# openfheorg/openfhe-boolean-circuit-evaluator

Measured on NVIDIA B200. Metric: bootstrapped gates/sec (STD128_OPT GINX), higher is better.
Workload: dtype u32

## Files before the change

### openfhe-boolean-circuit-evaluator_b200/csrc/common.hpp

```cpp
#pragma once
#include <cstddef>
#include <cstdint>

namespace bfhe {

using u8 = uint8_t;
using u16 = uint16_t;
using u32 = uint32_t;
using u64 = uint64_t;
using i32 = int32_t;
using i64 = int64_t;

struct DevConst {
  u32 Q, Q2;
  u32 qinv_neg;
  u32 unused_mu;
  u32 oneM;
  u32 Q8;
  u32 n, N, q, factor;
  u32 qKS, baseKS, dKS;
  u32 baseR, dR, dG, logBG;
  u32 ct_stride;
  u32 ninv, ninvs;
  u32 nM, nMs;
  u32 gate_const[9];
  u32 reserved_[3];
  u32 tw[32], tws[32], itw[32], itws[32];
};

struct DevGate {
  const u32 *in0;
  const u32 *in1;
  u32 *out;
  u32 op;
  u32 pad;
};

enum : u32 { OP_OR = 0, OP_AND = 1, OP_NOR = 2, OP_NAND = 3, OP_XOR_FAST = 4, OP_XNOR_FAST = 5, OP_XOR = 6, OP_XNOR = 7,
             OP_BOOTSTRAP = 8, OP_NEG0 = 0x100, OP_NEG1 = 0x200 };

struct LaunchInfo {
  int gates_per_cta;
  int ctas;
  size_t smem_bytes;
};

struct V2Bufs {
  const u32 *d_bk4 = nullptr;
  const u32 *d_tw2 = nullptr;
  const u32 *d_F = nullptr;
  const u32 *d_bkx = nullptr;
  const u32 *d_twx = nullptr;
};

int launch_blind_rotate(const DevConst &P, int method_ap, const DevGate *d_gates, int count, const u32 *d_bk,
                        const u32 *d_twl , const u32 *d_psiM,
                        u32 *d_ext , u32 *d_acc_dbg , int force_gates_per_cta,
                        void *stream, LaunchInfo *info, const V2Bufs *v2 = nullptr);
bool v2_supported(const DevConst &P, int method_ap);
int v2_set_attrs();
int launch_bk_permute_v2(const u32 *d_src, u32 *d_dst, size_t npoly, void *stream);
int cl2_max_gates();
int launch_bk_split_cl4(const u32 *d_src, u32 *d_dst, size_t npoly, void *stream);
int launch_blind_rotate_cl2(const DevConst &P, const DevGate *d_gates, int count, const V2Bufs &vb, u32 *d_ext, u32 *d_acc_dbg,
                            void *stream, LaunchInfo *info);
bool clx_supported(const DevConst &P, int method_ap);
size_t clx_tw_words();
int clx_set_attrs();
int clx_max_gates();
int clx_fast_gates();
int launch_bk_slice_clx(const u32 *d_src, u32 *d_dst, size_t npoly, int method_ap, void *stream);
int launch_blind_rotate_clx(const DevConst &P, int method_ap, const DevGate *d_gates, int count, const V2Bufs &vb, u32 *d_ext,
                            u32 *d_acc_dbg, void *stream, LaunchInfo *info);
struct PeerX {
  u32 *const *slabs = nullptr;
  const u32 *local_base = nullptr;
  u32 *const *flags = nullptr;
  u32 *counter = nullptr;
  const u32 *epoch = nullptr;
  u32 world = 1, rank = 0, index = 0, per_epoch = 1;
};
int launch_keyswitch(const DevConst &P, const u32 *d_ext, const DevGate *d_gates, int count, const void *d_ksk,
                     int ksk_elem_bytes, void *stream, const PeerX *px = nullptr);
int launch_peer_epoch_bump(u32 *epoch, void *stream);
int launch_peer_wait(const u32 *local_flags, const u32 *epoch, u32 world, u32 rank, int index, u32 per_epoch, u32 *err, void *stream);
int launch_peer_signal(const PeerX &px, void *stream);
int launch_eval_not(const DevConst &P, const u32 *const *d_in, u32 *const *d_out, int count, void *stream);
int launch_bk_convert(const DevConst &P, const u32 *d_coef, u32 *d_dev, size_t npoly, const u32 *d_twl, void *stream);
int launch_dbg_ntt(const DevConst &P, const u32 *d_a, const u32 *d_b, u32 *d_rt, u32 *d_prod, int npoly, const u32 *d_twl,
                   void *stream);
int launch_microbench(int which, u32 *d_sink, int iters, int *threads_total, int *ops_per_thread_iter, void *stream);
int blind_rotate_set_attrs();

}
```

### openfhe-boolean-circuit-evaluator_b200/csrc/engine.cu

```cuda
#include "engine.hpp"
#include "device.cuh"
#include <algorithm>
#include <cstdio>
#include <cstring>
#include <omp.h>

using namespace bfhe;

namespace bfhe {
static thread_local std::string g_err;
void set_error(const std::string &msg) { g_err = msg; }
int cuda_fail(cudaError_t e, const char *what) {
  set_error(std::string("CUDA error: ") + cudaGetErrorString(e) + " in " + what);
  return BFHE_ERR_CUDA;
}
}

extern "C" const char *bfhe_last_error(void) { return g_err.c_str(); }

static constexpr double SIGMA = 3.19;
static const GaussTable &gauss_table() {
  static const GaussTable t(SIGMA);
  return t;
}
// ... 159 lines not shown
          for (u32 g = 0; g < 2; g++) putf(at(1, 2 + g), 256 + 64 * k + 2 * lane + g);
          for (u32 g = 0; g < 4; g++) putf(at(1, 4 + g), 512 + 128 * k + 4 * lane + g);
        }
        for (u32 s5 = 0; s5 < 5; s5++)
          for (u32 t = 0; t < 256; t++) puti(8 + 256 * (size_t)s5 + t, (512u >> s5) + ((256 * k + t) >> (s5 + 1)));
      }
      ok = cudaMalloc(&c->d_twx, tx.size() * 4) == cudaSuccess && cudaMemcpy(c->d_twx, tx.data(), tx.size() * 4, cudaMemcpyHostToDevice) == cudaSuccess;
      c->v2.d_twx = c->d_twx;
    }
    int sms = 148;
    cudaDeviceGetAttribute(&sms, cudaDevAttrMultiProcessorCount, device);
    c->chunk = std::max<size_t>(1, bfhe_ctx::CHUNK / (4 * (size_t)sms)) * 4 * (size_t)sms;
    if (c->chunk > bfhe_ctx::CHUNK) c->chunk = bfhe_ctx::CHUNK;
    if (!ok) {
      cuda_fail(cudaGetLastError(), "bfhe_create: device allocation");
      bfhe_destroy(c);
      return nullptr;
    }
  }
  return c;
}

extern "C" void bfhe_destroy(bfhe_ctx *c) {
  if (!c) return;
  if (c->device >= 0) {
    cudaSetDevice(c->device);
    cudaDeviceSynchronize();
    for (auto &s : c->spans) { cudaEventDestroy(s.a); cudaEventDestroy(s.b); }
    cudaFree(c->d_bk); cudaFree(c->d_twl); cudaFree(c->d_psiM); cudaFree(c->d_ksk); cudaFree(c->d_gates); cudaFree(c->d_ext);
    cudaFree(c->d_tmp); cudaFree(c->d_ptr_in); cudaFree(c->d_ptr_out); cudaFree(c->e2e_slab);
    cudaFree(c->d_gates_b); cudaFree(c->d_ext_b);
    cudaFree(c->d_bk4); cudaFree(c->d_tw2); cudaFree(c->d_F);
    cudaFree(c->d_bkx); cudaFree(c->d_twx);
    for (int i = 0; i < 2; i++) {
      if (c->ev_br[i]) cudaEventDestroy(c->ev_br[i]);
      if (c->ev_ks[i]) cudaEventDestroy(c->ev_ks[i]);
    }
    if (c->ks_stream) cudaStreamDestroy(c->ks_stream);
    for (int i = 0; i < 2; i++) {
      if (c->h_gates[i]) cudaFreeHost(c->h_gates[i]);
      if (c->stage_ev[i]) cudaEventDestroy(c->stage_ev[i]);
    }
    if (c->own_stream) cudaStreamDestroy(c->own_stream);
  }
  delete c;
}

extern "C" int bfhe_get_params(const bfhe_ctx *c, bfhe_params *out) {
  if (!c || !out) return BFHE_ERR_ARG;
  *out = c->p;
  return BFHE_OK;
}
extern "C" int bfhe_set_stream(bfhe_ctx *c, void *s, int use_own) {
  if (!c || c->device < 0) return BFHE_ERR_STATE;
  c->stream = use_own ? c->own_stream : (cudaStream_t)s;
  return BFHE_OK;
}
extern "C" int bfhe_sync(bfhe_ctx *c) {
  if (!c || c->device < 0) { set_error("no device attached"); return BFHE_ERR_CUDA; }
  BFHE_CUDA(cudaStreamSynchronize(c->stream));
  return BFHE_OK;
}

extern "C" int bfhe_keygen(bfhe_ctx *c, uint64_t seed) {
  if (!c) return BFHE_ERR_ARG;
  SeedKey key;
// ... 117 lines not shown
    const size_t npoly = c->bk_words / N, slice = 1 << 15;
    u32 *d_coef = nullptr;
    BFHE_CUDA(cudaMalloc(&d_coef, std::min(npoly, slice) * N * 4));
    for (size_t p0 = 0; p0 < npoly; p0 += slice) {
      const size_t np = std::min(slice, npoly - p0);
      BFHE_CUDA(cudaMemcpyAsync(d_coef, c->bk_coef.data() + p0 * N, np * N * 4, cudaMemcpyHostToDevice, c->stream));
      int rc = launch_bk_convert(c->P, d_coef, c->d_bk + p0 * N, np, c->d_twl, c->stream);
      if (rc) return cuda_fail((cudaError_t)rc, "bk_convert");
      BFHE_CUDA(cudaStreamSynchronize(c->stream));
    }
    cudaFree(d_coef);
  }
  cudaFree(c->d_bk4); c->d_bk4 = nullptr; c->v2.d_bk4 = nullptr;
  if (c->d_tw2 && v2_supported(c->P, p.method == BFHE_AP)) {
    u32 *tmp = nullptr;
    BFHE_CUDA(cudaMalloc(&tmp, c->bk_words * 4));
    int rc = launch_bk_permute_v2(c->d_bk, tmp, c->bk_words / N, c->stream);
    if (rc) { cudaFree(tmp); return cuda_fail((cudaError_t)rc, "bk_permute_v2"); }
    if (cudaMalloc(&c->d_bk4, c->bk_words * 4) != cudaSuccess) { cudaFree(tmp); return cuda_fail(cudaGetLastError(), "cudaMalloc(d_bk4)"); }
    rc = launch_bk_split_cl4(tmp, c->d_bk4, c->bk_words / N, c->stream);
    if (rc) { cudaFree(tmp); return cuda_fail((cudaError_t)rc, "bk_split_cl4"); }
    cudaStreamSynchronize(c->stream);
    cudaFree(tmp);
    c->v2.d_bk4 = c->d_bk4;
  }
  cudaFree(c->d_bkx); c->d_bkx = nullptr; c->v2.d_bkx = nullptr;
  if (c->d_twx && clx_supported(c->P, p.method == BFHE_AP)) {
    BFHE_CUDA(cudaMalloc(&c->d_bkx, c->bk_words * 4));
    int rc = launch_bk_slice_clx(c->d_bk, c->d_bkx, c->bk_words / N, p.method == BFHE_AP, c->stream);
    if (rc) return cuda_fail((cudaError_t)rc, "bk_slice_clx");
    BFHE_CUDA(cudaStreamSynchronize(c->stream));
    c->v2.d_bkx = c->d_bkx;
  }
  {
    const u32 rowlen = c->ksk_elem_bytes == 2 ? 512 : p.ct_stride;
    if (c->ksk_elem_bytes == 2 && p.n + 1 > 512) { set_error("LWE dimension too large for the packed key-switch kernel"); return BFHE_ERR_ARG; }
    const size_t rows = (size_t)N * p.baseKS * p.dKS, bytes = rows * rowlen * c->ksk_elem_bytes;
    std::vector<u8> dev(bytes, 0);
    const size_t src_row = (size_t)(p.n + 1) * c->ksk_elem_bytes, dst_row = (size_t)rowlen * c->ksk_elem_bytes;
#pragma omp parallel for schedule(static)
    for (i64 i = 0; i < (i64)N; i++)
      for (u32 j = 0; j < p.baseKS; j++)
        for (u32 k = 0; k < p.dKS; k++) {
          const size_t s = (((size_t)i * p.baseKS + j) * p.dKS + k), d = (((size_t)i * p.dKS + k) * p.baseKS + j);
          std::memcpy(dev.data() + d * dst_row, c->ksk.data() + s * src_row, src_row);
        }
    BFHE_CUDA(cudaMalloc(&c->d_ksk, bytes));
    BFHE_CUDA(cudaMemcpy(c->d_ksk, dev.data(), bytes, cudaMemcpyHostToDevice));
  }
  c->dev_keys = true;
  return BFHE_OK;
}

extern "C" size_t bfhe_keyblob_size(const bfhe_ctx *c) {
  if (!c) return 0;
  return sizeof(KeyBlobHeader) + pad8((size_t)c->p.n * 4) + pad8(c->bk_words * 4) + pad8(c->ksk_elems * c->ksk_elem_bytes);
}
extern "C" int bfhe_export_keys(const bfhe_ctx *c, void *buf, size_t cap, int include_sk) {
  if (!c || !buf) return BFHE_ERR_ARG;
  if (!c->has_bt) { set_error("no keys to export"); return BFHE_ERR_STATE; }
  if (cap < bfhe_keyblob_size(c)) { set_error("export buffer too small"); return BFHE_ERR_ARG; }
  KeyBlobHeader h{};
  std::memcpy(h.magic, "BFHEKEY1", 8);
  const bfhe_params &p = c->p;
  h.version = 1; h.paramset = p.paramset; h.method = p.method; h.n = p.n; h.N = p.N; h.q = p.q;
  h.baseKS = p.baseKS; h.dKS = p.dKS; h.baseG = p.baseG; h.dG = p.dG; h.baseR = p.baseR; h.dR = p.dR;
// ... 435 lines not shown
```

### openfhe-boolean-circuit-evaluator_b200/csrc/engine.hpp

```cpp
#pragma once
#include "../../include/bfhe.h"
#include "common.hpp"
#include "hostmath.hpp"
#include <cuda_runtime.h>
#include <mutex>
#include <string>
#include <vector>

namespace bfhe {

void set_error(const std::string &msg);
int cuda_fail(cudaError_t e, const char *what);
#define BFHE_CUDA(call)                                                                                                \
  do {                                                                                                                 \
    cudaError_t _e = (call);                                                                                           \
    if (_e != cudaSuccess) return ::bfhe::cuda_fail(_e, #call);                                                        \
  } while (0)

struct ProfSpan {
  cudaEvent_t a, b;
  int kernel;
};

}

struct bfhe_ctx {
  bfhe_params p{};
  bfhe::DevConst P{};
  int device = -1;
  cudaStream_t own_stream = nullptr, stream = nullptr;
  bfhe::u64 psi = 0;
  bfhe::HostNtt hntt;

  std::vector<bfhe::i32> sk;
  std::vector<bfhe::i32> z;
  bool has_sk = false, has_bt = false;
  bool ofhe_have_bk = false, ofhe_have_ksk = false;
  std::vector<bfhe::u32> bk_coef;
  std::vector<bfhe::u8> ksk;
  bfhe::u32 ksk_elem_bytes = 4;
  bfhe::u64 bk_words = 0, ksk_elems = 0;

  bfhe::u32 *d_bk = nullptr, *d_twl = nullptr, *d_psiM = nullptr;
  void *d_ksk = nullptr;
  bfhe::u32 *d_bk4 = nullptr, *d_tw2 = nullptr, *d_F = nullptr;
  bfhe::u32 *d_bkx = nullptr, *d_twx = nullptr;
  bfhe::V2Bufs v2{};
  bool dev_keys = false;

  static constexpr size_t CHUNK = 32768;
  size_t chunk = CHUNK;
  bfhe::DevGate *d_gates = nullptr;
  bfhe::DevGate *d_gates_b = nullptr;
  bfhe::u32 *d_ext_b = nullptr;
  cudaStream_t ks_stream = nullptr;
  cudaEvent_t ev_br[2] = {nullptr, nullptr}, ev_ks[2] = {nullptr, nullptr};
  bfhe::DevGate *h_gates[2] = {nullptr, nullptr};
  cudaEvent_t stage_ev[2] = {nullptr, nullptr};
  int stage_next = 0;
  bfhe::u32 *d_ext = nullptr;
  bfhe::u32 *d_tmp = nullptr;
  size_t tmp_rows = 0;
  const bfhe::u32 **d_ptr_in = nullptr;
  bfhe::u32 **d_ptr_out = nullptr;
  size_t ptr_cap = 0;
  bfhe::u32 *e2e_slab = nullptr;
  size_t e2e_rows = 0;
  int force_g = 0;
  double form_cost_ms[4] = {0, 0, 0, 0};
  bool form_cost_measured = false;

  bool profiling = false;
  std::vector<bfhe::ProfSpan> spans;
  std::mutex mtx;
};

namespace bfhe {
int run_gate_list(bfhe_ctx *c, const DevGate *host_list, size_t count, u32 *acc_dbg_host);
int ensure_device_keys(bfhe_ctx *c);
// ... 2 lines not shown
```

### openfhe-boolean-circuit-evaluator_b200/csrc/kernels.cu

```cuda
#include "device.cuh"
#include <type_traits>
#include <cuda_runtime.h>
#include <cstdlib>

namespace bfhe {

constexpr int SOL_LAT_WIDE = 0x05, SOL_LAT_NARROW = 0x0a;

__device__ __forceinline__ u32 f_phys(u32 u) { return (u & ~31u) | ((u ^ (u >> 5)) & 31u); }
template <int E> struct Lay {
  static constexpr int C = E / 4;
  __device__ __forceinline__ static int swz(int tp) { return E == 32 ? (tp & 7) : ((tp >> 1) & 3); }
  __device__ __forceinline__ static int chunk_off(int tp, int c) { return E * tp + 4 * (c ^ swz(tp)); }
  __device__ __forceinline__ static int elem_off(int k, int lane) {
    if (E == 32) return 32 * k + 4 * ((lane >> 2) ^ (k & 7)) + (lane & 3);
    int j = lane & 15;
    return 16 * (2 * k + (lane >> 4)) + 4 * ((j >> 2) ^ (k & 3)) + (j & 3);
  }
};
template <int E> __device__ __forceinline__ void row_load(const u32 *buf, u32 (&x)[E], int lane) {
#pragma unroll
  for (int c = 0; c < E / 4; c++) {
    uint4 v = *reinterpret_cast<const uint4 *>(buf + Lay<E>::chunk_off(lane, c));
    x[4 * c] = v.x; x[4 * c + 1] = v.y; x[4 * c + 2] = v.z; x[4 * c + 3] = v.w;
// ... 85 lines not shown
  int B = B0;
  for (int T = 1; T < E; T *= 2) {
    const int NB = 2 * B;
    const bool last = 2 * T >= E;
    B = (last ? NB > MAXLAST : NB > 16) ? 2 : NB;
  }
  return B;
}

struct TwTabs {
  const u32 *fw, *fws, *iw, *iws;
};

template <int LOGN, bool PRE = false, int SOLW = 0, int SOLN = 0>
__device__ __forceinline__ void ntt_forward(u32 (&x)[(1 << LOGN) / 32], u32 *buf, const DevConst &P, const TwTabs &tt, int lane,
                                            const u32 *pre = nullptr) {
  constexpr int E = (1 << LOGN) / 32;
  const u32 Q = P.Q, Q2 = P.Q2;
  ct_pass<E, true, SOLW, PRE>(x, P.tw, P.tws, Q, Q2, nullptr, nullptr, 0, pre);
  if constexpr (LOGN & 1) {
    const bool up = lane & 16;
#pragma unroll
    for (int k = 0; k < E; k++) {
      u32 v = up ? mul_shoup(x[k], P.tw[16 + k], P.tws[16 + k], Q) : x[k];
      u32 o = __shfl_xor_sync(0xffffffffu, v, 16);
      x[k] = up ? (o - v + Q2) : (v + o);
    }
  }
  __syncwarp();
  col_store<E>(buf, x, lane);
  __syncwarp();
  row_load<E>(buf, x, lane);
  ct_pass<E, false, SOLN>(x, P.tw, P.tws, Q, Q2, tt.fw, tt.fws, lane);
}

template <int LOGN, bool PRE = false>
__device__ __forceinline__ void ntt_forward2(u32 (&xa)[(1 << LOGN) / 32], u32 (&xb)[(1 << LOGN) / 32], u32 *bufa, u32 *bufb, const DevConst &P,
                                             const TwTabs &tt, int lane, const u32 *prea = nullptr, const u32 *preb = nullptr) {
  constexpr int E = (1 << LOGN) / 32;
  static_assert((LOGN & 1) == 0, "even log2 N only");
  const u32 Q = P.Q, Q2 = P.Q2;
  ct_pass<E, true, 0, PRE>(xa, P.tw, P.tws, Q, Q2, nullptr, nullptr, 0, prea);
  ct_pass<E, true, 0, PRE>(xb, P.tw, P.tws, Q, Q2, nullptr, nullptr, 0, preb);
  __syncwarp();
  col_store<E>(bufa, xa, lane);
  col_store<E>(bufb, xb, lane);
  __syncwarp();
  row_load<E>(bufa, xa, lane);
  row_load<E>(bufb, xb, lane);
  ct_pass<E, false>(xa, P.tw, P.tws, Q, Q2, tt.fw, tt.fws, lane);
  ct_pass<E, false>(xb, P.tw, P.tws, Q, Q2, tt.fw, tt.fws, lane);
}

template <int LOGN, int B0>
__device__ __forceinline__ void ntt_inverse(u32 (&x)[(1 << LOGN) / 32], u32 *buf, const DevConst &P, const TwTabs &tt, int lane) {
  constexpr int E = (1 << LOGN) / 32;
  const u32 Q = P.Q;
  constexpr int ML = (LOGN & 1) ? 8 : 16;
  GsRun<E, 1, B0, false, ML>::run(x, P.itw, P.itws, Q, tt.iw, tt.iws, lane);
  constexpr int B1 = gs_out_bound(E, B0, ML);
  __syncwarp();
  row_store<E>(buf, x, lane);
  __syncwarp();
  col_load<E>(buf, x, lane);
  if constexpr (LOGN & 1) {
    static_assert(B1 <= 8, "bound");
    const bool up = lane & 16;
    const u32 off = B1 * Q;
#pragma unroll
    for (int k = 0; k < E; k++) {
      u32 o = __shfl_xor_sync(0xffffffffu, x[k], 16);
      u32 D = o - x[k] + off;
      x[k] = up ? mul_shoup(D, P.itw[16 + k], P.itws[16 + k], Q) : (x[k] + o);
    }
    constexpr int B2 = 2 * B1;
    GsRun<E, 1, B2, true, 32>::run(x, P.itw, P.itws, Q);
  } else {
    GsRun<E, 1, B1, true, 32>::run(x, P.itw, P.itws, Q);
  }
#pragma unroll
  for (int k = 0; k < E; k++) x[k] = csub(lazy_reduce(x[k], Q), Q);
}

__device__ __forceinline__ u32 brev(u32 x, int bits) { return __brev(x) >> (32 - bits); }
template <int DG, int LOGBG> constexpr u32 digit_offset() {
  u32 off = 0;
  for (int l = 0; l < DG; l++) off += (1u << (LOGBG - 1)) << (LOGBG * l);
  return off;
}

template <int LOGN, int DG, int LOGBG, int G, bool AP> struct BrCfg {
  static constexpr int N = 1 << LOGN, E = N / 32, C = E / 4, ROWS = 2 * DG;
  static constexpr int W = 2 * G, THREADS = 32 * W;
  static constexpr int NPAD = AP ? 1024 : 512;
  static constexpr size_t dct_words = (size_t)G * ROWS * N;
  static constexpr bool LUT = (LOGBG == 7 && LOGN == 10);
  static constexpr size_t lut_words = LUT ? (size_t)32 << LOGBG : 0;
  static constexpr size_t smem_bytes = (dct_words + 4 * N + (AP ? 0 : 2 * N) + lut_words) * 4 + (size_t)G * NPAD * 2;
};

template <int LOGN, int DG, int LOGBG, int G, bool AP>
__global__ void __launch_bounds__(64 * G, 1)
blind_rotate_kernel(const __grid_constant__ DevConst P, const DevGate *__restrict__ gates, int count,
                    const u32 *__restrict__ bk, const u32 *__restrict__ g_twl, const u32 *__restrict__ g_psiM,
                    u32 *__restrict__ ext, u32 *__restrict__ acc_dbg) {
  using Cfg = BrCfg<LOGN, DG, LOGBG, G, AP>;
  constexpr int N = Cfg::N, E = Cfg::E, C = Cfg::C, ROWS = Cfg::ROWS, W = Cfg::W, NPAD = Cfg::NPAD;
  constexpr u32 DIGIT_OFF = digit_offset<DG, LOGBG>();
  extern __shared__ __align__(128) unsigned char smem_raw[];
  u32 *dct = reinterpret_cast<u32 *>(smem_raw);
  u32 *s_tw = dct + Cfg::dct_words;
  u32 *s_psiM = s_tw + 4 * N;
  u32 *s_lut = s_psiM + (AP ? 0 : 2 * N);
  u16 *s_idx = reinterpret_cast<u16 *>(s_lut + Cfg::lut_words);

  const int tid = threadIdx.x, lane = tid & 31, warp = tid >> 5;
  const int g = warp >> 1, c = warp & 1;
  if constexpr (Cfg::LUT) {
    for (int i = tid; i < (int)Cfg::lut_words; i += Cfg::THREADS) {
      const u32 d = (u32)i >> 5;
      s_lut[i] = (u32)(((u64)P.tw[1] * ((d + P.Q - (1u << (LOGBG - 1))) % P.Q)) % P.Q);
    }
  }
  const int gate0 = blockIdx.x * G;
  const int gcount = min(G, count - gate0);
  const u32 Q = P.Q, q = P.q, n = P.n;

  for (int i = tid; i < 4 * N; i += Cfg::THREADS) s_tw[i] = g_twl[i];
  if (!AP)
    for (int u = tid; u < N; u += Cfg::THREADS) s_psiM[f_phys((u32)u)] = (g_psiM[2 * u] + (P.Q - P.oneM)) % P.Q;
  const TwTabs tt{s_tw, s_tw + N, s_tw + 2 * N, s_tw + 3 * N};

  __shared__ u32 s_b[G];
  for (int gg = 0; gg < gcount; gg++) {
    const DevGate dg = gates[gate0 + gg];
    const u32 gate = dg.op & 0xff;
    for (u32 i = tid; i <= n; i += Cfg::THREADS) {
      u32 x = dg.in0[i];
      if (dg.op & OP_NEG0) x = (i == n) ? (q / 4 + q - x) % q : (q - x) % q;
      u32 v;
      if (gate == OP_BOOTSTRAP) {
// ... 4 lines not shown
        v = (gate == OP_XOR_FAST || gate == OP_XNOR_FAST) ? (2 * (x + q - y)) % q : (x + y) % q;
      }
      if (i == n) s_b[gg] = v;
      else {
        u32 aneg = (q - v) % q;
        if (!AP) s_idx[gg * NPAD + i] = (u16)(aneg * P.factor);
        else {
          u32 a = aneg;
          for (u32 k = 0; k < P.dR; k++, a /= P.baseR) s_idx[gg * NPAD + i * P.dR + k] = (u16)(a % P.baseR);
        }
      }
    }
  }
  __syncthreads();

  const bool gvalid = g < gcount;
  u32 acc[E];
#pragma unroll
  for (int k = 0; k < E; k++) acc[k] = 0;
  if (gvalid && c == 1) {
    const u32 gate = gates[gate0 + g].op & 0xff;
    const u32 q1 = P.gate_const[gate == OP_BOOTSTRAP ? OP_AND : gate], q2 = (q1 + q / 2) % q;
    const u32 b = s_b[g], Q8 = P.Q8, Q8n = Q - P.Q8;
#pragma unroll
    for (int k = 0; k < E; k++) {
      const u32 idx = lane + 32 * k;
      if (idx % P.factor == 0) {
        const u32 t = (b + q - idx / P.factor) % q;
        const bool in = (q1 < q2) ? (t >= q1 && t < q2) : !(t >= q2 && t < q1);
        acc[k] = in ? Q8n : Q8;
      }
    }
  }

  const int nsteps = AP ? n * P.dR : n;
  bool pending = false;
  u32 *mybuf = dct + ((size_t)g * ROWS + c) * N;

  constexpr int GS = (W >= C) ? (W / C) : 1;
  const u32 eA = 2 * brev(lane, 5) + 1;
  constexpr bool PAIRED = Cfg::LUT && DG % 2 == 0 && G <= 2;
  constexpr bool KEY_HOIST = !AP && !PAIRED;

#ifdef BFHE_PHASE_TIMING
  long long tpt[5] = {0, 0, 0, 0, 0}, tq0 = clock64(), tq1;
#define PT_T(i) do { tq1 = clock64(); tpt[i] += tq1 - tq0; tq0 = tq1; } while (0)
#else
#define PT_T(i)
#endif
  for (int step = 0; step < nsteps; step++) {
    uint4 kr[2][ROWS][2];
#define BFHE_GX_LOAD(qc)                                     \
  do {                                                                                                                 \
    const u32 *kb_ = bk + (size_t)step * (2 * ROWS * 2) * N + ((qc) * 32 + lane) * 4;                                  \
    _Pragma("unroll") for (int s = 0; s < 2; s++)                                                                      \
      _Pragma("unroll") for (int r = 0; r < ROWS; r++)                                                                 \
        _Pragma("unroll") for (int cc = 0; cc < 2; cc++)                                                               \
          kr[s][r][cc] = __ldg(reinterpret_cast<const uint4 *>(kb_ + (size_t)((s * ROWS + r) * 2 + cc) * N));           \
  } while (0)
    constexpr int JN = (G + GS - 1) / GS;
    auto ap_key = [&](int gg, int qc) -> const u32 * {
      const u32 a0 = gg < gcount ? s_idx[gg * NPAD + step] : 0u;
      const u32 i = step / P.dR, k = step % P.dR;
      return bk + (((size_t)i * (P.baseR - 1) + (a0 ? a0 - 1 : 0u)) * P.dR + k) * (ROWS * 2) * N + (qc * 32 + lane) * 4;
    };
#define BFHE_AP_LOAD(buf, kb)                                                                                          \
  do {                                                                                                                 \
    const u32 *kb_ = (kb);                                                                                             \
    _Pragma("unroll") for (int r = 0; r < ROWS; r++)                                                                   \
      _Pragma("unroll") for (int cc = 0; cc < 2; cc++)                                                                 \
        kr[buf][r][cc] = __ldg(reinterpret_cast<const uint4 *>(kb_ + (size_t)(r * 2 + cc) * N));                        \
  } while (0)

    bool active = gvalid;
    if (AP && gvalid) active = s_idx[g * NPAD + step] != 0;
    if (active) {
      if (pending) {
        u32 x[E];
        row_load<E>(mybuf, x, lane);
        ntt_inverse<LOGN, AP ? 8 : 4>(x, mybuf, P, tt, lane);
#pragma unroll
        for (int k = 0; k < E; k++) acc[k] = AP ? x[k] : csub(acc[k] + x[k], Q);
      }
      u32 dp[E];
#pragma unroll
      for (int k = 0; k < E; k++) dp[k] = ((acc[k] < (Q >> 1)) ? acc[k] : acc[k] - Q) + DIGIT_OFF;
      if constexpr (PAIRED) {
#pragma unroll
        for (int l = 0; l < DG; l += 2) {
          u32 xa[E], xb[E], prea[E / 2], preb[E / 2];
#pragma unroll
          for (int k = 0; k < E; k++) {
            const u32 sh = dp[k] >> (LOGBG * l), da = sh & ((1u << LOGBG) - 1), db = (sh >> LOGBG) & ((1u << LOGBG) - 1);
            if (k >= E / 2) {
              prea[k - E / 2] = s_lut[(da << 5) + lane]; xa[k] = 0;
              preb[k - E / 2] = s_lut[(db << 5) + lane]; xb[k] = 0;
            } else {
              xa[k] = da + (Q - (1u << (LOGBG - 1)));
              xb[k] = db + (Q - (1u << (LOGBG - 1)));
            }
          }
          u32 *bufa = dct + ((size_t)g * ROWS + c + 2 * l) * N, *bufb = bufa + 2 * N;
          ntt_forward2<LOGN, true>(xa, xb, bufa, bufb, P, tt, lane, prea, preb);
          row_store<E>(bufa, xa, lane);
          row_store<E>(bufb, xb, lane);
        }
      } else {
#pragma unroll
      for (int l = 0; l < DG; l++) {
        u32 x[E], pre[Cfg::LUT ? E / 2 : 1];
#pragma unroll
        for (int k = 0; k < E; k++) {
          const u32 dgt = (dp[k] >> (LOGBG * l)) & ((1u << LOGBG) - 1);
          if (Cfg::LUT && k >= E / 2) { pre[Cfg::LUT ? k - E / 2 : 0] = s_lut[(dgt << 5) + lane]; x[k] = 0; }
          else x[k] = dgt + (Q - (1u << (LOGBG - 1)));
        }
        u32 *buf = dct + ((size_t)g * ROWS + c + 2 * l) * N;
        if (KEY_HOIST && l == DG - 1 && warp < C * GS) BFHE_GX_LOAD(warp % C);
        ntt_forward<LOGN, Cfg::LUT>(x, buf, P, tt, lane, pre);
        row_store<E>(buf, x, lane);
      }
      }
    } else if (KEY_HOIST && warp < C * GS) {
      BFHE_GX_LOAD(warp % C);
    }
    pending = pending || active;
    PT_T(0);
    if (AP && warp < C * GS) {
      BFHE_AP_LOAD(0, ap_key(warp / C, warp % C));
      if (JN > 1) BFHE_AP_LOAD(1, ap_key(warp / C + GS, warp % C));
    }
    if (!AP && !KEY_HOIST && warp < C * GS) BFHE_GX_LOAD(warp % C);
    __syncthreads();
    PT_T(1);

    for (int item = warp; item < C * GS; item += W) {
      const int qc = item % C, gs0 = item / C;
      if (!AP && item != warp) BFHE_GX_LOAD(qc);
      u32 eB[4];
#pragma unroll
      for (int r = 0; r < 4; r++) eB[r] = 2 * ((brev(r, 2) << (LOGN - 2)) | (brev(qc, LOGN - 7) << 5));

      if (AP && item != warp) {
        BFHE_AP_LOAD(0, ap_key(gs0, qc));
        if (JN > 1) BFHE_AP_LOAD(1, ap_key(gs0 + GS, qc));
      }
#pragma unroll
      for (int j = 0; j < JN; j++) {
        const int gg = gs0 + j * GS;
        const bool ap_active = AP && gg < gcount && s_idx[(gg < gcount ? gg : 0) * NPAD + step] != 0;
        if (gg >= gcount || (AP && !ap_active)) {
          if (AP && j + 2 < JN) { if ((j & 1) == 0) BFHE_AP_LOAD(0, ap_key(gs0 + (j + 2) * GS, qc)); else BFHE_AP_LOAD(1, ap_key(gs0 + (j + 2) * GS, qc)); }
          continue;
        }
        u32 fp[4], fn[4];
        if (!AP) {
          const u32 m = s_idx[gg * NPAD + step];
#pragma unroll
          for (int r = 0; r < 4; r++) {
            const u32 u = ((m * (eA + eB[r])) >> 1) & (N - 1);
            fp[r] = s_psiM[f_phys(u)];
            fn[r] = s_psiM[f_phys((0u - u) & (N - 1))];
          }
        }
        u32 *gd = dct + (size_t)gg * ROWS * N + Lay<E>::chunk_off(lane, qc);
        uint4 dv[ROWS];
#pragma unroll
        for (int r = 0; r < ROWS; r++) dv[r] = *reinterpret_cast<const uint4 *>(gd + (size_t)r * N);
#pragma unroll
        for (int cc = 0; cc < 2; cc++) {
          u32 out[4];
#pragma unroll
          for (int sl = 0; sl < 4; sl++) {
            u64 sp = 0, sn = 0;
#pragma unroll
            for (int r = 0; r < ROWS; r++) {
              const u32 dval = sl == 0 ? dv[r].x : sl == 1 ? dv[r].y : sl == 2 ? dv[r].z : dv[r].w;
              const uint4 kp = kr[AP ? (j & 1) : 0][r][cc];
              sp += (u64)dval * (sl == 0 ? kp.x : sl == 1 ? kp.y : sl == 2 ? kp.z : kp.w);
              if (!AP) {
                const uint4 kn = kr[AP ? 0 : 1][r][cc];
                sn += (u64)dval * (sl == 0 ? kn.x : sl == 1 ? kn.y : sl == 2 ? kn.z : kn.w);
              }
            }
            const u32 pp = redc(sp, Q, P.qinv_neg);
            if (AP) out[sl] = pp;
            else {
              const u32 pn = redc(sn, Q, P.qinv_neg);
              out[sl] = redc((u64)pp * fp[sl] + (u64)pn * fn[sl], Q, P.qinv_neg);
            }
          }
          *reinterpret_cast<uint4 *>(gd + (size_t)cc * N) = make_uint4(out[0], out[1], out[2], out[3]);
        }
        if (AP && j + 2 < JN) {
          if ((j & 1) == 0) BFHE_AP_LOAD(0, ap_key(gs0 + (j + 2) * GS, qc)); else BFHE_AP_LOAD(1, ap_key(gs0 + (j + 2) * GS, qc));
        }
      }
    }
    PT_T(2);
    __syncthreads();
    PT_T(3);
  }

  if (gvalid) {
    if (pending) {
      u32 x[E];
      row_load<E>(mybuf, x, lane);
      ntt_inverse<LOGN, AP ? 8 : 4>(x, mybuf, P, tt, lane);
#pragma unroll
      for (int k = 0; k < E; k++) acc[k] = AP ? x[k] : csub(acc[k] + x[k], Q);
    }
    const size_t gi = (size_t)gate0 + g;
    if (acc_dbg) {
#pragma unroll
      for (int k = 0; k < E; k++) acc_dbg[(gi * 2 + c) * N + lane + 32 * k] = acc[k];
    }
    u32 *e = ext + gi * (N + 4);
    const u64 qKS = P.qKS;
    if (c == 0) {
#pragma unroll
      for (int k = 0; k < E; k++) {
        const u32 j = lane + 32 * k;
        const u32 v = (j == 0) ? acc[k] : (acc[k] == 0 ? 0 : Q - acc[k]);
        const u32 pos = (j == 0) ? 0 : N - j;
        e[pos] = (qKS == Q) ? v : (u32)(((2 * (u64)v * qKS + Q) / (2 * (u64)Q)) % qKS);
// ... 407 lines not shown
  DevConst P{};
  int rc = 0;
  for (int G : {1, 2, 4}) {
    rc |= launch_br_g<LOGN, DG, LOGBG, false>(G, P, nullptr, 0, nullptr, nullptr, nullptr, nullptr, nullptr, 0, nullptr);
    rc |= launch_br_g<LOGN, DG, LOGBG, true>(G, P, nullptr, 0, nullptr, nullptr, nullptr, nullptr, nullptr, 0, nullptr);
  }
  rc |= launch_lat_inst<LOGN, DG, LOGBG, false>(P, nullptr, 0, nullptr, nullptr, nullptr, nullptr, nullptr, 0, nullptr);
  rc |= launch_lat_inst<LOGN, DG, LOGBG, true>(P, nullptr, 0, nullptr, nullptr, nullptr, nullptr, nullptr, 0, nullptr);
  return rc;
}
int blind_rotate_set_attrs() {
  int rc = br_attrs<10, 4, 7>();
  rc |= br_attrs<9, 3, 9>();
  rc |= v2_set_attrs();
  rc |= clx_set_attrs();
  return rc;
}

int launch_blind_rotate(const DevConst &P, int method_ap, const DevGate *d_gates, int count, const u32 *d_bk, const u32 *d_twl,
                        const u32 *d_psiM, u32 *d_ext, u32 *d_acc_dbg, int force_g, void *stream, LaunchInfo *info, const V2Bufs *v2) {
  if (count <= 0) return 0;
  cudaStream_t st = (cudaStream_t)stream;
  const bool have_cl2 = v2 && v2->d_bk4 && v2->d_tw2 && v2->d_F && v2_supported(P, method_ap);
  const bool have_clx = v2 && v2->d_bkx && v2->d_twx && (method_ap || v2->d_F) && clx_supported(P, method_ap);
  if (force_g == 128) return have_clx ? launch_blind_rotate_clx(P, method_ap, d_gates, count, *v2, d_ext, d_acc_dbg, stream, info) : (int)cudaErrorInvalidValue;
  if (force_g == 32) return have_cl2 ? launch_blind_rotate_cl2(P, d_gates, count, *v2, d_ext, d_acc_dbg, stream, info) : (int)cudaErrorInvalidValue;
  if (force_g != 0 && force_g != 1 && force_g != 2 && force_g != 4 && force_g != 8) return (int)cudaErrorInvalidValue;
  int dev = 0, sms = 148;
  cudaGetDevice(&dev);
  cudaDeviceGetAttribute(&sms, cudaDevAttrMultiProcessorCount, dev);
  if (force_g == 0 && have_clx && count <= clx_fast_gates()) return launch_blind_rotate_clx(P, method_ap, d_gates, count, *v2, d_ext, d_acc_dbg, stream, info);
  if (force_g == 0 && have_cl2 && count <= cl2_max_gates()) return launch_blind_rotate_cl2(P, d_gates, count, *v2, d_ext, d_acc_dbg, stream, info);
  const long lat_cost = (long)((count + sms - 1) / sms) * 222;
  const long thr_cost = (long)((count + 4 * sms - 1) / (4 * sms)) * 670;
  const bool lat = force_g == 8 || (force_g == 0 && lat_cost <= thr_cost);
  if (lat) {
    if (P.N == 1024 && P.dG == 4 && P.logBG == 7)
      return method_ap ? launch_lat_inst<10, 4, 7, true>(P, d_gates, count, d_bk, d_twl, d_psiM, d_ext, d_acc_dbg, st, info)
                       : launch_lat_inst<10, 4, 7, false>(P, d_gates, count, d_bk, d_twl, d_psiM, d_ext, d_acc_dbg, st, info);
    if (P.N == 512 && P.dG == 3 && P.logBG == 9)
      return method_ap ? launch_lat_inst<9, 3, 9, true>(P, d_gates, count, d_bk, d_twl, d_psiM, d_ext, d_acc_dbg, st, info)
                       : launch_lat_inst<9, 3, 9, false>(P, d_gates, count, d_bk, d_twl, d_psiM, d_ext, d_acc_dbg, st, info);
    return (int)cudaErrorInvalidValue;
  }
  int G = force_g > 0 ? force_g : 4;
  if (P.N == 1024 && P.dG == 4 && P.logBG == 7) {
    return method_ap ? launch_br_g<10, 4, 7, true>(G, P, d_gates, count, d_bk, d_twl, d_psiM, d_ext, d_acc_dbg, st, info)
                     : launch_br_g<10, 4, 7, false>(G, P, d_gates, count, d_bk, d_twl, d_psiM, d_ext, d_acc_dbg, st, info);
  }
  if (P.N == 512 && P.dG == 3 && P.logBG == 9) {
    return method_ap ? launch_br_g<9, 3, 9, true>(G, P, d_gates, count, d_bk, d_twl, d_psiM, d_ext, d_acc_dbg, st, info)
                     : launch_br_g<9, 3, 9, false>(G, P, d_gates, count, d_bk, d_twl, d_psiM, d_ext, d_acc_dbg, st, info);
  }
  return (int)cudaErrorInvalidValue;
}

__device__ __forceinline__ void peer_store(const PeerX &px, const u32 *out, int k, u32 v) {
  if (px.slabs == nullptr) return;
  const size_t off = (size_t)(out - px.local_base) + (size_t)k;
  for (u32 r = 0; r < px.world; r++)
    if (r != px.rank) px.slabs[r][off] = v;
}
__device__ __forceinline__ void st_release_sys(u32 *p, u32 v) { asm volatile("st.release.sys.global.u32 [%0], %1;" ::"l"(p), "r"(v) : "memory"); }
__device__ __forceinline__ u32 ld_acquire_sys(const u32 *p) {
  u32 v;
  asm volatile("ld.acquire.sys.global.u32 %0, [%1];" : "=r"(v) : "l"(p) : "memory");
  return v;
}
__device__ __forceinline__ void peer_publish(const PeerX &px, u32 total) {
  if (px.slabs == nullptr) return;
  __threadfence_system();
  __syncthreads();
  if (threadIdx.x == 0) {
    const u32 done = atomicAdd(px.counter, 1u) + 1u;
    if (done == total) {
      atomicExch(px.counter, 0u);
      __threadfence_system();
      const u32 v = *px.epoch * px.per_epoch + px.index + 1u;
      for (u32 r = 0; r < px.world; r++)
        if (r != px.rank) st_release_sys(px.flags[r] + px.rank, v);
    }
// ... 208 lines not shown
                                                                             const u32 *__restrict__ g_twl) {
  constexpr int N = 1 << LOGN, E = N / 32;
  __shared__ __align__(16) u32 s_tw[4 * N];
  __shared__ __align__(16) u32 s_buf[4][N];
  const int lane = threadIdx.x & 31, warp = threadIdx.x >> 5;
  for (int i = threadIdx.x; i < 4 * N; i += blockDim.x) s_tw[i] = g_twl[i];
  __syncthreads();
  const TwTabs tt{s_tw, s_tw + N, s_tw + 2 * N, s_tw + 3 * N};
  for (size_t p = (size_t)blockIdx.x * 4 + warp; p < npoly; p += (size_t)gridDim.x * 4) {
    u32 x[E];
#pragma unroll
    for (int k = 0; k < E; k++) x[k] = coef[p * N + lane + 32 * k];
    ntt_forward<LOGN>(x, s_buf[warp], P, tt, lane);
#pragma unroll
    for (int c = 0; c < E / 4; c++) {
      u32 o[4];
#pragma unroll
      for (int r = 0; r < 4; r++) o[r] = csub(mul_shoup(x[4 * c + r], P.nM, P.nMs, P.Q), P.Q);
      *reinterpret_cast<uint4 *>(dev + p * N + (c * 32 + lane) * 4) = make_uint4(o[0], o[1], o[2], o[3]);
    }
    __syncwarp();
  }
}
int launch_bk_convert(const DevConst &P, const u32 *d_coef, u32 *d_dev, size_t npoly, const u32 *d_twl, void *stream) {
  if (npoly == 0) return 0;
  int blocks = (int)((npoly + 3) / 4);
  if (blocks > 148 * 16) blocks = 148 * 16;
  if (P.N == 1024) bk_convert_kernel<10><<<blocks, 128, 0, (cudaStream_t)stream>>>(P, d_coef, d_dev, npoly, d_twl);
  else if (P.N == 512) bk_convert_kernel<9><<<blocks, 128, 0, (cudaStream_t)stream>>>(P, d_coef, d_dev, npoly, d_twl);
  else return (int)cudaErrorInvalidValue;
  return (int)cudaGetLastError();
}

template <int LOGN> __global__ void __launch_bounds__(32) dbg_ntt_kernel(const __grid_constant__ DevConst P, const u32 *__restrict__ a,
                                                                         const u32 *__restrict__ b, u32 *__restrict__ rt,
                                                                         u32 *__restrict__ prod, const u32 *__restrict__ g_twl) {
  constexpr int N = 1 << LOGN, E = N / 32;
  __shared__ __align__(16) u32 s_tw[4 * N];
  __shared__ __align__(16) u32 s_buf[N];
  const int lane = threadIdx.x;
  for (int i = lane; i < 4 * N; i += 32) s_tw[i] = g_twl[i];
  __syncwarp();
  const TwTabs tt{s_tw, s_tw + N, s_tw + 2 * N, s_tw + 3 * N};
  const size_t p = blockIdx.x;
  const u32 Q = P.Q;
  u32 x[E], y[E];
#pragma unroll
  for (int k = 0; k < E; k++) x[k] = a[p * N + lane + 32 * k];
  ntt_forward<LOGN>(x, s_buf, P, tt, lane);
#pragma unroll
  for (int k = 0; k < E; k++) y[k] = csub(lazy_reduce(x[k], Q), Q);
  {
    u32 z[E];
#pragma unroll
    for (int k = 0; k < E; k++) z[k] = y[k];
    __syncwarp();
    ntt_inverse<LOGN, 2>(z, s_buf, P, tt, lane);
#pragma unroll
    for (int k = 0; k < E; k++) rt[p * N + lane + 32 * k] = csub(mul_shoup(z[k], P.ninv, P.ninvs, Q), Q);
  }
  if (b) {
    u32 z[E];
#pragma unroll
    for (int k = 0; k < E; k++) z[k] = b[p * N + lane + 32 * k];
    __syncwarp();
    ntt_forward<LOGN>(z, s_buf, P, tt, lane);
// ... 55 lines not shown
```

### openfhe-boolean-circuit-evaluator_b200/host/circuit.cpp

```cpp
#include "../csrc/engine.hpp"
#include "netlist.hpp"
#include <algorithm>
#include <chrono>
#include <cstdio>
#include <cstdlib>
#include <cstring>
#include <dlfcn.h>
#include <queue>

using namespace bfhe;

namespace {

struct Id128 { char b[128]; };
struct NcclApi {
  void *h = nullptr;
  int (*GetUniqueId)(void *) = nullptr;
  int (*CommInitRank)(void **, int, Id128, int) = nullptr;
  int (*AllGather)(const void *, void *, size_t, int, void *, cudaStream_t) = nullptr;
  int (*Broadcast)(const void *, void *, size_t, int, int, void *, cudaStream_t) = nullptr;
  int (*CommDestroy)(void *) = nullptr;
  const char *(*GetErrorString)(int) = nullptr;
};
NcclApi g_nccl;
bool load_nccl() {
  if (g_nccl.h) return true;
  void *h = dlopen("libnccl.so.2", RTLD_NOW | RTLD_GLOBAL);
  if (!h) h = dlopen("libnccl.so", RTLD_NOW | RTLD_GLOBAL);
  if (!h) { set_error(std::string("cannot load NCCL: ") + dlerror()); return false; }
  g_nccl.GetUniqueId = (decltype(g_nccl.GetUniqueId))dlsym(h, "ncclGetUniqueId");
  g_nccl.CommInitRank = (decltype(g_nccl.CommInitRank))dlsym(h, "ncclCommInitRank");
  g_nccl.AllGather = (decltype(g_nccl.AllGather))dlsym(h, "ncclAllGather");
  g_nccl.Broadcast = (decltype(g_nccl.Broadcast))dlsym(h, "ncclBroadcast");
  g_nccl.CommDestroy = (decltype(g_nccl.CommDestroy))dlsym(h, "ncclCommDestroy");
  g_nccl.GetErrorString = (decltype(g_nccl.GetErrorString))dlsym(h, "ncclGetErrorString");
  if (!g_nccl.GetUniqueId || !g_nccl.CommInitRank || !g_nccl.AllGather || !g_nccl.Broadcast || !g_nccl.CommDestroy) {
    set_error("NCCL symbols missing");
    return false;
  }
  g_nccl.h = h;
  return true;
}
constexpr int NCCL_UINT32 = 3, NCCL_FLOAT32 = 7;

struct NotOp { uint32_t in_row, out_row, copy; };
struct Level {
  std::vector<bfhe_gate> gates;
  uint32_t first_row = 0;
  std::vector<NotOp> nots;
  bool sharded = true;
};
struct FormCosts {
  double cl4 = 1.05, cl2 = 1.55, lat = 2.36, thr = 7.6, exchange = exchange_default();
  bool measured = false;
  static double exchange_default() { const char *m = std::getenv("BFHE_EXCHANGE"); return m && std::strcmp(m, "nccl") == 0 ? 0.05 : 0.015; }
};
inline bool is_single(GateKind k) {
  return k == GateKind::AND || k == GateKind::OR || k == GateKind::NAND || k == GateKind::NOR || k == GateKind::XOR_FAST || k == GateKind::XNOR_FAST;
}
inline bool is_boot(GateKind k) { return is_single(k) || k == GateKind::XOR; }
inline uint32_t op_of(GateKind k) {
  switch (k) {
  case GateKind::AND: return BFHE_AND;
  case GateKind::OR: return BFHE_OR;
  case GateKind::NAND: return BFHE_NAND;
  case GateKind::NOR: return BFHE_NOR;
  case GateKind::XOR_FAST: return BFHE_XOR_FAST;
  default: return BFHE_XNOR_FAST;
  }
}

}

struct bfhe_circuit {
  bfhe_ctx *ctx = nullptr;
  Netlist nl;
  Netlist nl_file;
  bool loaded = false;
  bool plaintext = false, encrypted = false, verify = false;
  bool planned_verify = false;
  int rank = 0, world = 1;
  void *comm = nullptr;

  bool planned = false;
  std::vector<uint32_t> topo;
  std::vector<uint32_t> wire_row;
// ... 1143 lines not shown
```

Baseline: 86560.

## Fold top gadget digit into a precomputed bootstrapping key for GINX throughput kernel

Precomputes a folded bootstrapping key in which the top decomposition digit is expressed through the lower digits and the full accumulator, using powers of the inverse base. The GINX throughput kernel then runs one fewer forward NTT per step: it keeps an NTT-domain copy of the accumulator and updates it alongside the output. The paired two-NTT path is removed, and the cost-model constants that choose between kernel forms are retuned. In exchange the kernel needs an extra key buffer and extra per-step accumulator bookkeeping, and the scheme relies on the digit range covering the centred accumulator.

```diff
diff --git a/openfhe-boolean-circuit-evaluator_b200/csrc/common.hpp b/openfhe-boolean-circuit-evaluator_b200/csrc/common.hpp
--- a/openfhe-boolean-circuit-evaluator_b200/csrc/common.hpp
+++ b/openfhe-boolean-circuit-evaluator_b200/csrc/common.hpp
@@ -51,6 +51,7 @@
   const u32 *d_F = nullptr;
   const u32 *d_bkx = nullptr;
   const u32 *d_twx = nullptr;
+  const u32 *d_bkf = nullptr;
 };
 
 int launch_blind_rotate(const DevConst &P, int method_ap, const DevGate *d_gates, int count, const u32 *d_bk,
@@ -87,6 +88,8 @@
 int launch_peer_signal(const PeerX &px, void *stream);
 int launch_eval_not(const DevConst &P, const u32 *const *d_in, u32 *const *d_out, int count, void *stream);
 int launch_bk_convert(const DevConst &P, const u32 *d_coef, u32 *d_dev, size_t npoly, const u32 *d_twl, void *stream);
+bool bk_fold_supported(const DevConst &P, int method_ap);
+int launch_bk_fold(const DevConst &P, const u32 *d_bk, u32 *d_bkf, size_t nsteps, void *stream);
 int launch_dbg_ntt(const DevConst &P, const u32 *d_a, const u32 *d_b, u32 *d_rt, u32 *d_prod, int npoly, const u32 *d_twl,
                    void *stream);
 int launch_microbench(int which, u32 *d_sink, int iters, int *threads_total, int *ops_per_thread_iter, void *stream);
diff --git a/openfhe-boolean-circuit-evaluator_b200/csrc/engine.cu b/openfhe-boolean-circuit-evaluator_b200/csrc/engine.cu
--- a/openfhe-boolean-circuit-evaluator_b200/csrc/engine.cu
+++ b/openfhe-boolean-circuit-evaluator_b200/csrc/engine.cu
@@ -215,6 +215,7 @@
     cudaFree(c->d_gates_b); cudaFree(c->d_ext_b);
     cudaFree(c->d_bk4); cudaFree(c->d_tw2); cudaFree(c->d_F);
     cudaFree(c->d_bkx); cudaFree(c->d_twx);
+    cudaFree(c->d_bkf);
     for (int i = 0; i < 2; i++) {
       if (c->ev_br[i]) cudaEventDestroy(c->ev_br[i]);
       if (c->ev_ks[i]) cudaEventDestroy(c->ev_ks[i]);
@@ -398,6 +399,14 @@
     BFHE_CUDA(cudaStreamSynchronize(c->stream));
     c->v2.d_bkx = c->d_bkx;
   }
+  cudaFree(c->d_bkf); c->d_bkf = nullptr; c->v2.d_bkf = nullptr;
+  if (bk_fold_supported(c->P, p.method == BFHE_AP)) {
+    BFHE_CUDA(cudaMalloc(&c->d_bkf, c->bk_words * 4));
+    int rc = launch_bk_fold(c->P, c->d_bk, c->d_bkf, p.n, c->stream);
+    if (rc) return cuda_fail((cudaError_t)rc, "bk_fold");
+    BFHE_CUDA(cudaStreamSynchronize(c->stream));
+    c->v2.d_bkf = c->d_bkf;
+  }
   {
     const u32 rowlen = c->ksk_elem_bytes == 2 ? 512 : p.ct_stride;
     if (c->ksk_elem_bytes == 2 && p.n + 1 > 512) { set_error("LWE dimension too large for the packed key-switch kernel"); return BFHE_ERR_ARG; }
diff --git a/openfhe-boolean-circuit-evaluator_b200/csrc/engine.hpp b/openfhe-boolean-circuit-evaluator_b200/csrc/engine.hpp
--- a/openfhe-boolean-circuit-evaluator_b200/csrc/engine.hpp
+++ b/openfhe-boolean-circuit-evaluator_b200/csrc/engine.hpp
@@ -45,6 +45,7 @@
   void *d_ksk = nullptr;
   bfhe::u32 *d_bk4 = nullptr, *d_tw2 = nullptr, *d_F = nullptr;
   bfhe::u32 *d_bkx = nullptr, *d_twx = nullptr;
+  bfhe::u32 *d_bkf = nullptr;
   bfhe::V2Bufs v2{};
   bool dev_keys = false;
 
diff --git a/openfhe-boolean-circuit-evaluator_b200/csrc/kernels.cu b/openfhe-boolean-circuit-evaluator_b200/csrc/kernels.cu
--- a/openfhe-boolean-circuit-evaluator_b200/csrc/kernels.cu
+++ b/openfhe-boolean-circuit-evaluator_b200/csrc/kernels.cu
@@ -141,24 +141,6 @@
   __syncwarp();
   row_load<E>(buf, x, lane);
   ct_pass<E, false, SOLN>(x, P.tw, P.tws, Q, Q2, tt.fw, tt.fws, lane);
-}
-
-template <int LOGN, bool PRE = false>
-__device__ __forceinline__ void ntt_forward2(u32 (&xa)[(1 << LOGN) / 32], u32 (&xb)[(1 << LOGN) / 32], u32 *bufa, u32 *bufb, const DevConst &P,
-                                             const TwTabs &tt, int lane, const u32 *prea = nullptr, const u32 *preb = nullptr) {
-  constexpr int E = (1 << LOGN) / 32;
-  static_assert((LOGN & 1) == 0, "even log2 N only");
-  const u32 Q = P.Q, Q2 = P.Q2;
-  ct_pass<E, true, 0, PRE>(xa, P.tw, P.tws, Q, Q2, nullptr, nullptr, 0, prea);
-  ct_pass<E, true, 0, PRE>(xb, P.tw, P.tws, Q, Q2, nullptr, nullptr, 0, preb);
-  __syncwarp();
-  col_store<E>(bufa, xa, lane);
-  col_store<E>(bufb, xb, lane);
-  __syncwarp();
-  row_load<E>(bufa, xa, lane);
-  row_load<E>(bufb, xb, lane);
-  ct_pass<E, false>(xa, P.tw, P.tws, Q, Q2, tt.fw, tt.fws, lane);
-  ct_pass<E, false>(xb, P.tw, P.tws, Q, Q2, tt.fw, tt.fws, lane);
 }
 
 template <int LOGN, int B0>
@@ -205,6 +187,7 @@
   static constexpr size_t dct_words = (size_t)G * ROWS * N;
   static constexpr bool LUT = (LOGBG == 7 && LOGN == 10);
   static constexpr size_t lut_words = LUT ? (size_t)32 << LOGBG : 0;
+  static constexpr bool FOLD = LUT && !AP;
   static constexpr size_t smem_bytes = (dct_words + 4 * N + (AP ? 0 : 2 * N) + lut_words) * 4 + (size_t)G * NPAD * 2;
 };
 
@@ -216,6 +199,10 @@
   using Cfg = BrCfg<LOGN, DG, LOGBG, G, AP>;
   constexpr int N = Cfg::N, E = Cfg::E, C = Cfg::C, ROWS = Cfg::ROWS, W = Cfg::W, NPAD = Cfg::NPAD;
   constexpr u32 DIGIT_OFF = digit_offset<DG, LOGBG>();
+  constexpr bool FOLD = Cfg::FOLD;
+  static_assert(!FOLD || (DIGIT_OFF >= (SOLINAS_Q + 1) / 2 && (u64)DIGIT_OFF + (SOLINAS_Q - 3) / 2 < (1ull << (LOGBG * DG))),
+                "the digits do not cover the centred accumulator: the top digit cannot be folded into the key");
+  constexpr int ND = FOLD ? DG - 1 : DG;
   extern __shared__ __align__(128) unsigned char smem_raw[];
   u32 *dct = reinterpret_cast<u32 *>(smem_raw);
   u32 *s_tw = dct + Cfg::dct_words;
@@ -286,6 +273,16 @@
       }
     }
   }
+  if (FOLD && gvalid) {
+    u32 x[E];
+#pragma unroll
+    for (int k = 0; k < E; k++) x[k] = acc[k];
+    u32 *abuf = dct + ((size_t)g * ROWS + 2 * (DG - 1) + c) * N;
+    ntt_forward<LOGN>(x, abuf, P, tt, lane);
+#pragma unroll
+    for (int k = 0; k < E; k++) x[k] = mul_shoup(x[k], P.ninv, P.ninvs, Q);
+    row_store<E>(abuf, x, lane);
+  }
 
   const int nsteps = AP ? n * P.dR : n;
   bool pending = false;
@@ -293,8 +290,7 @@
 
   constexpr int GS = (W >= C) ? (W / C) : 1;
   const u32 eA = 2 * brev(lane, 5) + 1;
-  constexpr bool PAIRED = Cfg::LUT && DG % 2 == 0 && G <= 2;
-  constexpr bool KEY_HOIST = !AP && !PAIRED;
+  constexpr bool KEY_HOIST = !AP;
 
 #ifdef BFHE_PHASE_TIMING
   long long tpt[5] = {0, 0, 0, 0, 0}, tq0 = clock64(), tq1;
@@ -339,29 +335,8 @@
       u32 dp[E];
 #pragma unroll
       for (int k = 0; k < E; k++) dp[k] = ((acc[k] < (Q >> 1)) ? acc[k] : acc[k] - Q) + DIGIT_OFF;
-      if constexpr (PAIRED) {
-#pragma unroll
-        for (int l = 0; l < DG; l += 2) {
-          u32 xa[E], xb[E], prea[E / 2], preb[E / 2];
-#pragma unroll
-          for (int k = 0; k < E; k++) {
-            const u32 sh = dp[k] >> (LOGBG * l), da = sh & ((1u << LOGBG) - 1), db = (sh >> LOGBG) & ((1u << LOGBG) - 1);
-            if (k >= E / 2) {
-              prea[k - E / 2] = s_lut[(da << 5) + lane]; xa[k] = 0;
-              preb[k - E / 2] = s_lut[(db << 5) + lane]; xb[k] = 0;
-            } else {
-              xa[k] = da + (Q - (1u << (LOGBG - 1)));
-              xb[k] = db + (Q - (1u << (LOGBG - 1)));
-            }
-          }
-          u32 *bufa = dct + ((size_t)g * ROWS + c + 2 * l) * N, *bufb = bufa + 2 * N;
-          ntt_forward2<LOGN, true>(xa, xb, bufa, bufb, P, tt, lane, prea, preb);
-          row_store<E>(bufa, xa, lane);
-          row_store<E>(bufb, xb, lane);
-        }
-      } else {
-#pragma unroll
-      for (int l = 0; l < DG; l++) {
+#pragma unroll
+      for (int l = 0; l < ND; l++) {
         u32 x[E], pre[Cfg::LUT ? E / 2 : 1];
 #pragma unroll
         for (int k = 0; k < E; k++) {
@@ -370,10 +345,9 @@
           else x[k] = dgt + (Q - (1u << (LOGBG - 1)));
         }
         u32 *buf = dct + ((size_t)g * ROWS + c + 2 * l) * N;
-        if (KEY_HOIST && l == DG - 1 && warp < C * GS) BFHE_GX_LOAD(warp % C);
+        if (KEY_HOIST && l == ND - 1 && warp < C * GS) BFHE_GX_LOAD(warp % C);
         ntt_forward<LOGN, Cfg::LUT>(x, buf, P, tt, lane, pre);
         row_store<E>(buf, x, lane);
-      }
       }
     } else if (KEY_HOIST && warp < C * GS) {
       BFHE_GX_LOAD(warp % C);
@@ -384,7 +358,6 @@
       BFHE_AP_LOAD(0, ap_key(warp / C, warp % C));
       if (JN > 1) BFHE_AP_LOAD(1, ap_key(warp / C + GS, warp % C));
     }
-    if (!AP && !KEY_HOIST && warp < C * GS) BFHE_GX_LOAD(warp % C);
     __syncthreads();
     PT_T(1);
 
@@ -445,6 +418,11 @@
             }
           }
           *reinterpret_cast<uint4 *>(gd + (size_t)cc * N) = make_uint4(out[0], out[1], out[2], out[3]);
+          if constexpr (FOLD) {
+            const uint4 a = dv[ROWS - 2 + cc];
+            *reinterpret_cast<uint4 *>(gd + (size_t)(ROWS - 2 + cc) * N) =
+                make_uint4(lazy_reduce(a.x + out[0], Q), lazy_reduce(a.y + out[1], Q), lazy_reduce(a.z + out[2], Q), lazy_reduce(a.w + out[3], Q));
+          }
         }
         if (AP && j + 2 < JN) {
           if ((j & 1) == 0) BFHE_AP_LOAD(0, ap_key(gs0 + (j + 2) * GS, qc)); else BFHE_AP_LOAD(1, ap_key(gs0 + (j + 2) * GS, qc));
@@ -918,7 +896,7 @@
   if (force_g == 0 && have_clx && count <= clx_fast_gates()) return launch_blind_rotate_clx(P, method_ap, d_gates, count, *v2, d_ext, d_acc_dbg, stream, info);
   if (force_g == 0 && have_cl2 && count <= cl2_max_gates()) return launch_blind_rotate_cl2(P, d_gates, count, *v2, d_ext, d_acc_dbg, stream, info);
   const long lat_cost = (long)((count + sms - 1) / sms) * 222;
-  const long thr_cost = (long)((count + 4 * sms - 1) / (4 * sms)) * 670;
+  const long thr_cost = (long)((count + 4 * sms - 1) / (4 * sms)) * 597;
   const bool lat = force_g == 8 || (force_g == 0 && lat_cost <= thr_cost);
   if (lat) {
     if (P.N == 1024 && P.dG == 4 && P.logBG == 7)
@@ -931,8 +909,10 @@
   }
   int G = force_g > 0 ? force_g : 4;
   if (P.N == 1024 && P.dG == 4 && P.logBG == 7) {
-    return method_ap ? launch_br_g<10, 4, 7, true>(G, P, d_gates, count, d_bk, d_twl, d_psiM, d_ext, d_acc_dbg, st, info)
-                     : launch_br_g<10, 4, 7, false>(G, P, d_gates, count, d_bk, d_twl, d_psiM, d_ext, d_acc_dbg, st, info);
+    if (method_ap) return launch_br_g<10, 4, 7, true>(G, P, d_gates, count, d_bk, d_twl, d_psiM, d_ext, d_acc_dbg, st, info);
+    static_assert(BrCfg<10, 4, 7, 4, false>::FOLD, "the GINX throughput kernel of this shape reads the folded key");
+    if (!v2 || !v2->d_bkf) return (int)cudaErrorInvalidValue;
+    return launch_br_g<10, 4, 7, false>(G, P, d_gates, count, v2->d_bkf, d_twl, d_psiM, d_ext, d_acc_dbg, st, info);
   }
   if (P.N == 512 && P.dG == 3 && P.logBG == 9) {
     return method_ap ? launch_br_g<9, 3, 9, true>(G, P, d_gates, count, d_bk, d_twl, d_psiM, d_ext, d_acc_dbg, st, info)
@@ -1207,6 +1187,43 @@
   return (int)cudaGetLastError();
 }
 
+struct FoldConst {
+  u32 w[8];
+};
+template <int DG> __global__ void __launch_bounds__(256) bk_fold_kernel(const u32 *__restrict__ bk, u32 *__restrict__ bkf, size_t total, u32 N, u32 Q,
+                                                                        const FoldConst F) {
+  constexpr int ROWS = 2 * DG, T = DG - 1;
+  for (size_t i = (size_t)blockIdx.x * blockDim.x + threadIdx.x; i < total; i += (size_t)gridDim.x * blockDim.x) {
+    const size_t cs = i % (2 * (size_t)N), c = (i / (2 * (size_t)N)) & 1, ss = i / (4 * (size_t)N);
+    const size_t base = ss * ROWS * 2 * N + cs;
+    const u64 top = bk[base + (c + 2 * T) * 2 * N];
+#pragma unroll
+    for (int l = 0; l < T; l++) {
+      const size_t o = base + (c + 2 * l) * 2 * N;
+      bkf[o] = (u32)(((u64)bk[o] + Q - top * F.w[l] % Q) % Q);
+    }
+    bkf[base + (c + 2 * T) * 2 * N] = (u32)(top * F.w[T] % Q);
+  }
+}
+static u64 powmod_q(u64 b, u64 e, u64 Q) {
+  u64 r = 1;
+  for (b %= Q; e; e >>= 1, b = b * b % Q)
+    if (e & 1) r = r * b % Q;
+  return r;
+}
+bool bk_fold_supported(const DevConst &P, int method_ap) { return !method_ap && P.N == 1024 && P.dG == 4 && P.logBG == 7; }
+int launch_bk_fold(const DevConst &P, const u32 *d_bk, u32 *d_bkf, size_t nsteps, void *stream) {
+  if (!bk_fold_supported(P, 0)) return (int)cudaErrorInvalidValue;
+  constexpr int DG = 4, T = DG - 1;
+  FoldConst F{};
+  const u64 Q = P.Q, binv = powmod_q(1ull << P.logBG, Q - 2, Q);
+  for (int l = 0; l < T; l++) F.w[l] = (u32)powmod_q(binv, T - l, Q);
+  F.w[T] = (u32)((u64)P.N * powmod_q(binv, T, Q) % Q);
+  const size_t total = nsteps * 2 * 2 * 2 * (size_t)P.N;
+  bk_fold_kernel<DG><<<148 * 8, 256, 0, (cudaStream_t)stream>>>(d_bk, d_bkf, total, P.N, P.Q, F);
+  return (int)cudaGetLastError();
+}
+
 template <int LOGN> __global__ void __launch_bounds__(32) dbg_ntt_kernel(const __grid_constant__ DevConst P, const u32 *__restrict__ a,
                                                                          const u32 *__restrict__ b, u32 *__restrict__ rt,
                                                                          u32 *__restrict__ prod, const u32 *__restrict__ g_twl) {
diff --git a/openfhe-boolean-circuit-evaluator_b200/host/circuit.cpp b/openfhe-boolean-circuit-evaluator_b200/host/circuit.cpp
--- a/openfhe-boolean-circuit-evaluator_b200/host/circuit.cpp
+++ b/openfhe-boolean-circuit-evaluator_b200/host/circuit.cpp
@@ -51,7 +51,7 @@
   bool sharded = true;
 };
 struct FormCosts {
-  double cl4 = 1.05, cl2 = 1.55, lat = 2.36, thr = 7.6, exchange = exchange_default();
+  double cl4 = 1.05, cl2 = 1.55, lat = 2.36, thr = 6.1, exchange = exchange_default();
   bool measured = false;
   static double exchange_default() { const char *m = std::getenv("BFHE_EXCHANGE"); return m && std::strcmp(m, "nccl") == 0 ? 0.05 : 0.015; }
 };
```

New measurement: 97770, median of 6. +12.9%, better.
